# sykefi/syke-pic

Measured on AMD Instinct MI355X. Metric: IFCB images/sec, resnet50 224x224 infer step, higher is better.
Workload: dtype f16; 1 GPU; resnet50_infer_b256x1_224x224x3_50cls_head256-128; per_gpu_batch=256, global_batch=256, precision=calibrated, parallelism=dp1

## Files before the change

### include/sykepic_hip.h

```cpp
#ifndef SYKEPIC_HIP_H
#define SYKEPIC_HIP_H

#include <stdint.h>

#ifdef __cplusplus
extern "C" {
#endif

#define SPK_OK 0
#define SPK_ERR_ARG (-1)
#define SPK_ERR_HIP (-2)
#define SPK_ERR_KEY (-3)
#define SPK_ERR_UNSUPPORTED (-4)
#define SPK_ERR_STATE (-5)

#define SPK_OP_CONV 1
#define SPK_OP_MAXPOOL 2
#define SPK_OP_GAVGPOOL 3
#define SPK_OP_LINEAR 4
#define SPK_OP_DROPOUT 5
#define SPK_OP_DWCONV 6
#define SPK_OP_SE 7

#define SPK_ACT_NONE 0
// ... 135 lines not shown
int spk_op_conv_group_dgrad(const void* dy_dev, const float* w_dev, void* dx_dev, int accumulate, int n, int h, int w,
                            int c, int groups, int stride, void* hip_stream);
int spk_op_conv_group_wgrad(const void* x_dev, const void* dy_dev, float* dw_dev, int n, int h, int w, int c, int groups,
                            int stride, void* hip_stream);
int spk_op_pw_fp8(const void* x_dev, int a_fp8, const float* w_dev, void* y_dev, int out_fp8, const void* res_dev,
                  const float* bn_scale_dev, const float* bn_bias_dev, const float* gate_dev, int hw, int m_rows, int cin,
                  int cout, int act, float a_scale, float y_scale, void* hip_stream);
int spk_op_conv1x1(const void* x_dev, const float* w_dev, const float* bn_scale_dev, const float* bn_bias_dev,
                   const void* res_dev, void* y_dev, int n, int h, int w, int cin, int cout, int stride, int relu,
                   int split, int cfg, void* hip_stream);
int spk_op_conv1x1_num_configs(void);
int spk_op_conv3x3(const void* x_dev, const float* w_dev, const float* bn_scale_dev, const float* bn_bias_dev,
                   const void* res_dev, void* y_dev, int n, int h, int w, int cin, int cout, int relu, int split, int cfg,
                   void* hip_stream);
int spk_op_conv3x3_num_configs(void);
int spk_op_bottleneck(const void* x_dev, const float* w1_dev, const float* w2_dev, const float* w3_dev, const float* s1_dev,
                      const float* b1_dev, const float* s2_dev, const float* b2_dev, const float* s3_dev, const float* b3_dev,
                      void* y_dev, int n, int h, int w, int cm, int fused, int iters, float* ms_out, void* stream,
                      unsigned long long* stamps_dev ,
                      const float* wz_dev, const float* sz_dev, const float* bz_dev, void* z_dev, int coutz);
int spk_op_conv1x1_chain(const void* x, const float* w, const float* bn_scale, const float* bn_bias, const void* res,
                         void* y, const float* wz, const float* bnz_scale, const float* bnz_bias, void* z, int n, int h,
                         int wd, int cin, int cout, int coutz, int relu, int reluz, void* stream);
int spk_op_conv1x1_dual(const void* x, const float* w1, const float* s1, const float* b1, const void* x2, const float* w2,
                        const float* s2, const float* b2, void* y, int n, int ho, int wo, int cin, int h2, int w2d, int cin2,
                        int cout, int stride2, int relu, int split, int cfg, void* stream);
int spk_op_zero_sum_round(const float* w_dev, const float* mu_dev, float* out_dev, int64_t rows, int row_len,
                          int mu_period, void* stream);
int spk_op_dwconv(const void* x_dev, const float* w_dev, const float* bn_scale_dev, const float* bn_bias_dev, void* y_dev,
                  float* pool_dev, int n, int h, int w, int channels, int k, int stride, int act, int lds, void* hip_stream);
// ... 103 lines not shown
```

### syke-pic_amd/csrc/asan_driver.hip

```cpp
#include "model.h"
#include "tune_table.h"
#include <algorithm>
#include <cmath>
#include <cstdio>
#include <cstdlib>
#include <cstring>
#include <sstream>
#include <string>
#include <vector>

static int g_fail = 0;
#define EXPECT(c) do { if (!(c)) { fprintf(stderr, "asan_driver: %s:%d: %s\n", __FILE__, __LINE__, #c); ++g_fail; } } while (0)

static spk_layer_desc conv(const char* name, const char* bn, int cin, int cout, int k, int s, int p, int src, int dst,
                           int res, int relu, int child) {
  spk_layer_desc d;
  memset(&d, 0, sizeof d);
  d.kind = SPK_OP_CONV; d.cin = cin; d.cout = cout; d.k = k; d.stride = s; d.pad = p; d.relu = relu;
  d.src = src; d.dst = dst; d.res = res; d.child = child;
  snprintf(d.name, sizeof d.name, "%s", name);
  snprintf(d.bn, sizeof d.bn, "%s", bn);
  return d;
}

// ... 90 lines not shown
    spk_tune_store((TuneTag)l.tag, l.v.data(), v, true);
  }
  EXPECT(std::count(tags, tags + TUNE_NTAGS, true) == 6);
  std::vector<TuneLine> back = read_tune_lines(tmp);
  auto by_text = [](const TuneLine& x, const TuneLine& y) { return x.text < y.text; };
  std::sort(lines.begin(), lines.end(), by_text);
  std::sort(back.begin(), back.end(), by_text);
  EXPECT(back.size() == lines.size());
  for (size_t i = 0; i < lines.size() && i < back.size(); ++i) EXPECT(back[i].text == lines[i].text);

  const std::vector<std::vector<int>> fresh = {
      {2, 1, 0, 5, 9, 9, 64, 64, 3, 1, 16, 1, 0, 6, 5}, {1, 9, 9, 64, 64, 1, 0, 1, 5, -1}, {1, 9, 9, 64, 18, 18, 64, 128, 1, 2, 5, 17},
      {2, 9, 9, 64, 64, 5, 13}, {9, 9, 64, 0, 64, 5, 0}, {9, 64, 5, 2}, {81, 64, 64, 3, 1, 0, 1, 64064, 1}};
  for (int t = 0; t < (int)fresh.size(); ++t) spk_tune_store((TuneTag)t, fresh[t].data(), fresh[t].data() + kTuneSchemas[t].n_key, true);
  spk_tune_store(TUNE_DW, dk, &one, true);
  EXPECT(read_tune_lines(tmp).size() == lines.size() + fresh.size());
  use_cache(tmp.c_str());
  for (int t = 0; t < (int)fresh.size(); ++t) {
    int v[2] = {-1000, -1000};
    EXPECT(spk_tune_find((TuneTag)t, fresh[t].data(), v));
    for (int i = 0; i < kTuneSchemas[t].n_val; ++i) EXPECT(v[i] == fresh[t][kTuneSchemas[t].n_key + i]);
  }
  EXPECT(look(TUNE_DW, {0, 64, 28, 28, 240, 5, 1}) == -1000);
  EXPECT(spk_tune_detail::table().map.size() == lines.size() + fresh.size());
  remove(tmp.c_str());
}

int main(int argc, char** argv) {
  int ndev = 0;
  const bool gpu = hipGetDeviceCount(&ndev) == hipSuccess && ndev > 0;
  printf("asan_driver: %d GPU(s)\n", gpu ? ndev : 0);

  spk_model* m = nullptr;
  EXPECT(spk_model_create(nullptr, 0, 3, 10, 0, &m) != SPK_OK);
  EXPECT(strlen(spk_last_error()) > 0);
  EXPECT(spk_model_num_params(nullptr) == 0);
  spk_model_destroy(nullptr);
  {
    float f[4] = {0};
// ... 69 lines not shown
  }

  const std::string path = std::string(getenv("TMPDIR") ? getenv("TMPDIR") : "/tmp") + "/spk_asan_tune_cache.txt";
  std::string seed = argc > 1 ? argv[1] : std::string(argv[0]);
  if (argc <= 1) seed = seed.substr(0, seed.find_last_of('/') + 1) + "../../../sykepic_hip/tune_seed_gfx950.txt";
  tuner_table_checks(path + ".rt", seed);
  std::string fixture;
  if (FILE* f = fopen(path.c_str(), "w")) {
    fprintf(f, "conv 0 1 1 256 14 14 256 256 3 1 16 0 0 4 3\n");
    fprintf(f, "pw1x1 2 14 14 256 1024 1 1 1 256 7\n");
    fprintf(f, "pw2 1 14 14 256 28 28 512 1024 1 2 256 5\n");
    fprintf(f, "c3 1 14 14 256 256 256 2\n");
    fprintf(f, "chain 14 14 256 0 256 64 0\n");
    fprintf(f, "bneck 14 256 8 1\n");
    fprintf(f, "wgrad 6272 256 256 3 1 0 13 128128 1\n");
    fprintf(f, "pw1x1 2 14 14 256 2048 1 1 1 256 99999\n");
    fprintf(f, "pw1x1 2 14 14 256 2048 1 1 1 256 -2\n");
    fprintf(f, "pw2 1 14 14 256 28 28 512 2048 1 2 256 %d\n", kPwNumCfgs);
    fprintf(f, "pw2 1 14 14 256 28 28 512 2048 1 2 256 -1\n");
    fprintf(f, "c3 1 14 14 256 512 256 %d\n", kC3NumCfgs);
    fprintf(f, "chain 14 14 256 0 512 64 2\n");
    fprintf(f, "bneck 28 128 8 3\n");
    fprintf(f, "c3 1 14 14\n");
    fprintf(f, "bneck 28 128 8\n");
    fprintf(f, "bneck 28 128 8 1 1\n");
    fprintf(f, "chain 14 14 256 0 512 64 1x\n");
    fprintf(f, "wgrad 6272 256 512 3 1 0 13 128128 99999999999\n");
    fprintf(f, "# bneck 28 128 8 2\n#bneck 28 128 8 2\n");
    fprintf(f, "conv x y z\n\n,,,,\nbneck\nbneckx 28 128 8 2\n");
    for (int i = 0; i < 3000; ++i) fputc('9', f);
// ... 3 lines not shown
    fprintf(f, "wgrad 1 2 3\n");
    fprintf(f, "c3 2 7 7 512 512 128 13");
    fclose(f);
    for (const TuneLine& l : read_tune_lines(path)) fixture += l.text;
  }
  use_cache(path.c_str());
  int dma = -1;
  EXPECT(look(TUNE_CONV, {0, 1, 1, 256, 14, 14, 256, 256, 3, 1, 16, 0, 0}, &dma) == 4 && dma == 3);
  EXPECT(look(TUNE_PW1, {2, 14, 14, 256, 1024, 1, 1, 1, 256}) == 7);
  EXPECT(look(TUNE_PW2, {1, 14, 14, 256, 28, 28, 512, 1024, 1, 2, 256}) == 5);
  EXPECT(look(TUNE_C3, {1, 14, 14, 256, 256, 256}) == 2);
  EXPECT(look(TUNE_CHAIN, {14, 14, 256, 0, 256, 64}) == 0);
  EXPECT(look(TUNE_BNECK, {14, 256, 8}) == 1);
  EXPECT(look(TUNE_WGRAD, {6272, 256, 256, 3, 1, 0, 13, 128128}) == 1);
  EXPECT(look(TUNE_C3, {2, 7, 7, 512, 512, 128}) == 13);
  EXPECT(look(TUNE_PW1, {2, 14, 14, 256, 2048, 1, 1, 1, 256}) == -1000);
  EXPECT(look(TUNE_PW2, {1, 14, 14, 256, 28, 28, 512, 2048, 1, 2, 256}) == -1000);
  EXPECT(look(TUNE_C3, {1, 14, 14, 256, 512, 256}) == -1000);
  EXPECT(look(TUNE_CHAIN, {14, 14, 256, 0, 512, 64}) == -1000);
  EXPECT(look(TUNE_BNECK, {28, 128, 8}) == -1000);
  EXPECT(look(TUNE_WGRAD, {6272, 256, 512, 3, 1, 0, 13, 128128}) == -1000);
  EXPECT(spk_tune_detail::table().map.size() == 8);
  setenv("SPK_AUTOTUNE", "0", 1);
  const int n = 1, h = 8, wd = 8, cin = 128, cout = 128, M = n * h * wd;
  bf16_t *x = nullptr, *y = nullptr, *wp = nullptr;
  float* sb = nullptr;
  if (gpu) {
    EXPECT(hipMalloc(&x, (size_t)M * cin * 2) == hipSuccess && hipMalloc(&y, (size_t)M * 256 * 2) == hipSuccess);
    EXPECT(hipMalloc(&wp, (size_t)256 * 9 * cin * 4) == hipSuccess && hipMalloc(&sb, (size_t)2 * 256 * 4) == hipSuccess);
    (void)hipMemset(x, 0, (size_t)M * cin * 2);
    (void)hipMemset(wp, 0, (size_t)256 * 9 * cin * 4);
    (void)hipMemset(sb, 0, (size_t)2 * 256 * 4);
  }
  ConvArgs a;
  memset(&a, 0, sizeof a);
  a.cfg = a.dma = -1; a.cls_ph = a.cls_pw = -1;
  a.x = x; a.w = wp; a.y = y; a.scale = sb; a.bias = sb ? sb + cout : nullptr;
// ... 29 lines not shown
```

### syke-pic_amd/csrc/model.h

```cpp
#pragma once
#include "../../include/sykepic_hip.h"
#include "spk_common.h"

#include <string>
#include <unordered_map>
#include <vector>

enum ParamKind { PK_CONV_W = 1, PK_BN_W, PK_BN_B, PK_BN_MEAN, PK_BN_VAR, PK_BN_NBT, PK_FC_W, PK_FC_B,
                 PK_SE_W, PK_SE_B };

struct Param {
  std::string key;
  int kind = 0, layer = -1, dtype = 0, ndim = 0;
  int64_t shape[4] = {1, 1, 1, 1};
  int64_t numel = 0;
  bool trainable = false;
  int requires_grad = 0;
  int group = -1;
  size_t off = 0;
  long step = 0;
  double mu_product = 1.0;
};

struct TDim {
// ... 2 lines not shown
  int c_log = 0;
};

struct Layer {
  spk_layer_desc d;
  int mode = 0;
  int groups = 1;
  int kpad = 0;
  int p_w = -1, p_g = -1, p_b = -1, p_mean = -1, p_var = -1, p_nbt = -1;
  int p_w2 = -1, p_b2 = -1;
  int cin_p = 0, cout_p = 0;
  size_t wpack_off = 0, sb_off = 0;
  size_t wpw_off = 0;
  bool pw_ok = false;
  bool c3_ok = false;
  int dual_src = -1;
  int fused_into = -1;
  bool dual_ok = false;
  size_t wdual_off = 0;
  size_t sdual_off = 0;
  int chain_next = -1;
  int chained_by = -1;
  bool chained_now_h[2] = {false, false};
  int bn_c2 = -1, bn_c3 = -1;
  int bn_head = -1;
  bool bneck_now_h[2] = {false, false};
  bool btail_now_h[2] = {false, false};
  size_t mu_off = 0;
  int gate_conv = -1;
  int gate_from = -1;
// ... 154 lines not shown
```

### syke-pic_amd/csrc/model.hip

```cpp
#include "../../include/sykepic_hip.h"
#include "spk_common.h"
#include "model.h"
#include "tune_table.h"

#include <algorithm>
#include <cmath>
#include <cstdio>
#include <cstdlib>
#include <cstring>

static thread_local std::string g_err;

void spk_set_error(const std::string& s) { g_err = s; }

#define HIP_TRY(expr)                                                                   \
  do {                                                                                  \
    hipError_t e_ = (expr);                                                             \
    if (e_ != hipSuccess) {                                                             \
      spk_set_error(std::string(#expr) + ": " + hipGetErrorString(e_));                 \
      return SPK_ERR_HIP;                                                               \
    }                                                                                   \
  } while (0)

#define SPK_TRY(expr)              \
// ... 258 lines not shown
      L.wpack_off = wpack;
      wpack += (size_t)2 * L.cout_p * L.kpad;
      L.pw_ok = L.mode == CONV_MODE_GENERIC && L.d.k == 1 && L.d.pad == 0 && L.cin_p == L.d.cin && L.cout_p == L.d.cout &&
                L.d.cin % 64 == 0 && L.d.cout % 64 == 0 && L.kpad == L.d.cin && L.d.relu != SPK_ACT_HSWISH;
      if (L.pw_ok) {
        L.wpw_off = wpack;
        wpack += (size_t)2 * L.d.cout * L.d.cin;
      }
      L.c3_ok = L.mode == CONV_MODE_GENERIC && L.d.k == 3 && L.d.stride == 1 && L.d.pad == 1 && L.cin_p == L.d.cin &&
                L.cout_p == L.d.cout && L.d.cin % 64 == 0 &&
                (L.d.cout % 256 == 0 || (L.bn_head >= 0 && L.d.cout % 128 == 0)) && L.d.relu != SPK_ACT_HSWISH;
      if (L.c3_ok || (L.bn_head >= 0 && L.d.k == 3)) {
        L.wpw_off = wpack;
        wpack += (size_t)2 * L.d.cout * 9 * L.d.cin;
      }
    } else {
      continue;
    }
    L.sb_off = sb;
    sb += (size_t)2 * L.cout_p;
  }
  size_t wdual = 0, sdual = 0;
  for (size_t i = 0; i < m->layers.size(); ++i) {
    Layer& L = m->layers[i];
    if (L.d.kind != SPK_OP_CONV || !L.pw_ok || L.d.res < 0 || L.d.stride != 1) continue;
    for (size_t j = 0; j < m->layers.size(); ++j) {
      Layer& D = m->layers[j];
      if (D.d.kind != SPK_OP_CONV || D.d.dst != L.d.res || !D.pw_ok || !D.side_branch || D.d.relu != 0 || D.d.res >= 0 ||
          D.d.cout != L.d.cout || D.fused_into >= 0)
        continue;
// ... 297 lines not shown
      r = pack_stem3(m, L);
    else if (L.mode == CONV_MODE_GENERIC && (L.cin_p != L.d.cin || L.cout_p != L.d.cout))
      r = spk_launch_pack_padded(wsrc, m->wpack + L.wpack_off, L.d.cout, L.d.k * L.d.k, L.d.cin, L.cout_p,
                                 L.cin_p, m->infer_dt, layer_split(m, L), m->stream);
    else
      r = spk_launch_pack_weights(wsrc, m->wpack + L.wpack_off, L.d.cout, L.d.k, L.d.k, L.d.cin,
                                  L.mode, m->infer_dt, layer_split(m, L), m->stream);
    if (r) return fail(SPK_ERR_HIP, "pack_weights launch failed");
    if (L.pw_ok && m->infer_dt == DT_F16 &&
        spk_launch_pack_pw(wsrc, nullptr, m->wpack + L.wpw_off, L.d.cout, L.d.cin, DT_F16, layer_split(m, L) ? 2 : 1,
                           m->stream))
      return fail(SPK_ERR_HIP, "pack_pw launch failed");
    if ((L.c3_ok || (L.bn_head >= 0 && L.d.k == 3)) && m->infer_dt == DT_F16 &&
        spk_launch_pack_c3(wsrc, m->wpack + L.wpw_off, L.d.cout, L.d.cin, layer_split(m, L) ? 2 : 1, m->stream))
      return fail(SPK_ERR_HIP, "pack_c3 launch failed");
  }
  {
    size_t tmp_floats = 0;
    for (Layer& L : m->layers) {
      L.dual_ok = false;
      if (L.dual_src < 0 || m->infer_dt != DT_F16) continue;
      const Layer& D = m->layers[L.dual_src];
      if ((layer_split(m, L) != 0) != (layer_split(m, D) != 0)) continue;
      tmp_floats = std::max(tmp_floats, (size_t)L.d.cout * (L.d.cin + D.d.cin));
    }
    float* wcat = nullptr;
    float* mucat = nullptr;
    bool dual_zs = false;
    for (const Layer& L : m->layers) dual_zs |= L.dual_src >= 0 && layer_zero_sum(m, L) && layer_zero_sum(m, m->layers[L.dual_src]);
    if (tmp_floats) HIP_TRY(hipMalloc((void**)&wcat, tmp_floats * 4 * (dual_zs ? 2 : 1) + (dual_zs ? 16384 * 4 : 0)));
// ... 568 lines not shown
    return SPK_OK;
  }
  static const bool use_c3 = !getenv("SPK_C3") || atoi(getenv("SPK_C3")) != 0;
  if (use_c3 && L.c3_ok && a.dt == DT_F16 && !a.res_lo && !a.y_lo && !a.cin_s && !a.cout_s) {
    C3Args q;
    memset(&q, 0, sizeof q);
    q.x = a.x; q.wp = m->wpack + L.wpw_off; q.y = a.y; q.scale = a.scale; q.shift = a.bias;
    q.N = nb; q.H = in.h; q.W = in.w; q.Cin = a.Cin; q.Cout = a.Cout; q.M = a.M; q.relu = a.relu; q.dt = DT_F16;
    q.nb = a.splitw ? 2 : 1;
    q.x_bytes = a.x_bytes; q.y_bytes = (unsigned)((size_t)a.M * a.Cout * 2);
    q.wp_bytes = (unsigned)((size_t)a.Cout * 9 * a.Cin * 2 * q.nb);
    q.res = a.res;
    const int r = spk_conv3x3_launch(q, m->stream);
    if (r == 0) return SPK_OK;
    if (r != -3) return fail(SPK_ERR_HIP, std::string("3x3 conv launch failed for ") + L.d.name);
  }
  if (spk_conv_launch(a, L.mode, m->stream, nullptr))
    return fail(SPK_ERR_HIP, std::string("conv launch failed for ") + L.d.name);
  return SPK_OK;
}

static int dw_forced() {
  static const int v = getenv("SPK_DW_LDS") ? atoi(getenv("SPK_DW_LDS")) : -1;
  return v;
}

template <class F>
static int dw_choose(int et, int nb, int h, int w, int c, int k, int s, hipStream_t st, F run, const int* chunks) {
  if (dw_forced() >= 0) {
    const int v = dw_forced();
// ... 648 lines not shown
```

### syke-pic_amd/csrc/ops_abi.hip

```cpp
#include "model.h"
#include "train_effnet.h"

#include <algorithm>
#include <cstring>
#include <vector>

static int ofail(int code, const std::string& msg) {
  spk_set_error(msg);
  return code;
}

namespace {
struct Scratch {
  std::vector<void*> p;
  ~Scratch() { for (void* q : p) (void)hipFree(q); }
  template <typename T> T* get(size_t count) {
    void* q = nullptr;
    if (hipMalloc(&q, (count ? count : 1) * sizeof(T)) != hipSuccess) return nullptr;
    p.push_back(q);
    return (T*)q;
  }
};
bool stem_shape(int cin, int cout, int k, int stride, int pad) {
  return cin <= 4 && k == 7 && stride == 2 && pad == 3 && cout == 64;
// ... 353 lines not shown
    memset(&q, 0, sizeof q);
    q.x = (const bf16_t*)x; q.wp = wp; q.y = (bf16_t*)y; q.scale = bn_scale; q.shift = bn_bias;
    q.N = n; q.H = h; q.W = wd; q.Cin = cin; q.Cout = cout; q.M = M; q.relu = relu; q.dt = DT_F16; q.nb = split ? 2 : 1;
    q.x_bytes = (unsigned)((size_t)M * cin * 2);
    q.y_bytes = (unsigned)((size_t)M * cout * 2);
    q.wp_bytes = (unsigned)((size_t)cout * 9 * cin * 2 * q.nb);
    q.res = (const bf16_t*)res;
    r = spk_c3_launch(q, cfg, s);
    if (r == -3) return ofail(SPK_ERR_UNSUPPORTED, "this configuration does not fit the problem");
  }
  if (r) return ofail(SPK_ERR_HIP, "conv3x3 launch failed");
  if (hipStreamSynchronize(s) != hipSuccess) return ofail(SPK_ERR_HIP, "conv3x3 kernel failed");
  return SPK_OK;
}
extern "C" int spk_op_conv3x3_num_configs(void) { return spk_c3_num_configs(); }

extern "C" int spk_op_bottleneck(const void* x, const float* w1, const float* w2, const float* w3, const float* s1,
                                 const float* b1, const float* s2, const float* b2, const float* s3, const float* b3, void* y,
                                 int n, int h, int wd, int cm, int fused, int iters, float* ms_out, void* stream,
                                 unsigned long long* stamps_dev, const float* wz, const float* sz, const float* bz, void* z,
                                 int coutz) {
  if (!x || !w1 || !w2 || !w3 || !s1 || !b1 || !s2 || !b2 || !s3 || !b3 || !y || n < 1 || h < 1 || wd < 1 || x == y)
    return ofail(SPK_ERR_ARG, "op_bottleneck: bad arguments");
  if (cm % 64) return ofail(SPK_ERR_UNSUPPORTED, "mid channels must be a multiple of 64");
  hipStream_t s = (hipStream_t)stream;
  const int c4 = 4 * cm, M = n * h * wd;
  if ((size_t)M * c4 * 2 >= 0x80000000ull) return ofail(SPK_ERR_UNSUPPORTED, "op_bottleneck: an operand of 2 GiB or more");
  Scratch sc;
  bf16_t* p1 = sc.get<bf16_t>((size_t)cm * c4);
  bf16_t* p2 = sc.get<bf16_t>((size_t)9 * cm * cm);
// ... 643 lines not shown
```

### syke-pic_amd/csrc/spk_common.h

```cpp
#pragma once
#include <hip/hip_runtime.h>
#include <stdint.h>
#include <stddef.h>
#include <atomic>

static inline bool spk_lds_limit_once(std::atomic<unsigned long long>& mask, const void* kernel, int bytes) {
  int dev = 0;
  if (hipGetDevice(&dev) != hipSuccess) return false;
  const unsigned long long bit = dev >= 0 && dev < 64 ? 1ull << dev : 0ull;
  if (mask.load(std::memory_order_acquire) & bit) return true;
  if (hipFuncSetAttribute(kernel, hipFuncAttributeMaxDynamicSharedMemorySize, bytes) != hipSuccess) return false;
  mask.fetch_or(bit, std::memory_order_release);
  return true;
}

typedef unsigned short bf16_t;

typedef __attribute__((ext_vector_type(8))) __bf16 bf16x8_t;
typedef __attribute__((ext_vector_type(4))) float f32x4_t;
typedef __attribute__((ext_vector_type(4))) unsigned int u32x4_t;
typedef __attribute__((ext_vector_type(2))) unsigned int u32x2_t;

__device__ __forceinline__ float bf16_to_f32(bf16_t v) {
  return __builtin_bit_cast(float, ((unsigned int)v) << 16);
// ... 143 lines not shown
struct C3Args {
  const bf16_t* x;
  const bf16_t* wp;
  bf16_t* y;
  const float* scale;
  const float* shift;
  int N, H, W, Cin, Cout, M;
  int relu, dt, nb;
  unsigned int x_bytes, y_bytes, wp_bytes;
  const bf16_t* res;
};
int spk_c3_num_configs();
int spk_c3_launch(const C3Args& a, int cfg, hipStream_t s);
int spk_launch_pack_c3(const float* w_ohwi, bf16_t* out, int cout, int cin, int nb, hipStream_t s);
int spk_conv3x3_launch(const C3Args& a, hipStream_t s);

struct BneckArgs {
  const bf16_t* x;
  bf16_t* y;
  const bf16_t* w1;
  const bf16_t* w2;
  const bf16_t* w3;
  const float *s1, *b1, *s2, *b2, *s3, *b3;
  int N, H, W, C4, CM;
  unsigned int x_bytes;
  const bf16_t* y1;
  const bf16_t* wz;
  bf16_t* z;
  const float *sz, *bz;
  int Coutz;
// ... 140 lines not shown
```

### syke-pic_amd/csrc/tune_table.h

```cpp
#pragma once
#include <hip/hip_runtime.h>
#include <algorithm>
#include <array>
#include <climits>
#include <cstdio>
#include <cstdlib>
#include <cstring>
#include <map>
#include <mutex>

constexpr int kPwNumCfgs = 18;
constexpr int kC3NumCfgs = 14;

struct TuneSchema { const char* tag; int n_key, n_pos, n_val, val_min, val_max; };
enum TuneTag { TUNE_CONV, TUNE_PW1, TUNE_PW2, TUNE_C3, TUNE_CHAIN, TUNE_BNECK, TUNE_WGRAD, TUNE_DW, TUNE_NTAGS };
constexpr TuneSchema kTuneSchemas[TUNE_NTAGS] = {
    {"conv", 13, 3, 2, INT_MIN, INT_MAX},
    {"pw1x1", 9, 8, 1, -1, kPwNumCfgs - 1},
    {"pw2", 11, 10, 1, 0, kPwNumCfgs - 1},
    {"c3", 6, 5, 1, -1, kC3NumCfgs - 1},
    {"chain", 6, 5, 1, 0, 1},
    {"bneck", 3, 2, 1, 0, 2},
    {"wgrad", 8, -1, 1, INT_MIN, INT_MAX},
    {nullptr, 7, -1, 1, 0, 1},
};

inline const char* spk_tune_cache_path() {
  const char* e = getenv("SPK_TUNE_CACHE");
  return e && *e && strcmp(e, "off") ? e : nullptr;
}
inline bool spk_autotune_on() {
  static const bool v = !getenv("SPK_AUTOTUNE") || atoi(getenv("SPK_AUTOTUNE")) != 0;
  return v;
}
inline int spk_tune_log() {
  static const int v = getenv("SPK_TUNE_LOG") ? (atoi(getenv("SPK_TUNE_LOG")) > 1 ? atoi(getenv("SPK_TUNE_LOG")) : 1) : 0;
  return v;
}

// ... 136 lines not shown
```

### syke-pic_amd/sykepic_hip/lib.py

```python

import ctypes as C
import os
from pathlib import Path

_HERE = Path(__file__).resolve().parent
LIB_PATH = Path(os.environ.get("SYKEPIC_HIP_LIB", _HERE / "libsykepic_hip.so"))


class LayerDesc(C.Structure):
    _fields_ = [
        ("kind", C.c_int32), ("cin", C.c_int32), ("cout", C.c_int32), ("k", C.c_int32),
        ("stride", C.c_int32), ("pad", C.c_int32), ("relu", C.c_int32), ("src", C.c_int32),
        ("dst", C.c_int32), ("res", C.c_int32), ("child", C.c_int32), ("p", C.c_float),
        ("name", C.c_char * 96), ("bn", C.c_char * 96),
    ]


class OptimDesc(C.Structure):
    _fields_ = [
        ("kind", C.c_int32), ("lr", C.c_float * 3), ("beta1", C.c_float), ("beta2", C.c_float),
        ("eps", C.c_float), ("weight_decay", C.c_float), ("momentum", C.c_float),
        ("grad_scale", C.c_float), ("alpha", C.c_float), ("momentum_decay", C.c_float),
        ("lr_decay", C.c_float), ("initial_accumulator_value", C.c_float),
    ]
# ... 101 lines not shown
    "spk_op_mbconv_eval_geometry": (C.c_int, [C.c_int] * 5 + [C.POINTER(C.c_int)]),
    "spk_op_linear": (C.c_int, [_P] * 4 + [C.c_int] * 3 + [_P]),
    "spk_op_linear_backward": (C.c_int, [_P] * 6 + [C.c_int] * 4 + [_P]),
    "spk_op_softmax": (C.c_int, [_P, _P, C.c_int, C.c_int, C.c_float, _P]),
    "spk_op_cross_entropy": (C.c_int, [_P, _P, C.c_int, C.c_int, _P, _P, _P]),
    "spk_op_cross_entropy_ex": (C.c_int, [_P, _P, C.c_int, C.c_int, _P, C.c_float, _P, _P, _P, _P]),
    "spk_op_cross_entropy_pair": (C.c_int, [_P, _P, _P, C.c_float, C.c_int, C.c_int, _P, C.c_float, _P, _P, _P, _P]),
    "spk_op_maxpool": (C.c_int, [_P] * 3 + [C.c_int] * 8 + [_P]),
    "spk_op_maxpool_backward": (C.c_int, [_P] * 3 + [C.c_int] * 8 + [_P]),
    "spk_op_gavgpool": (C.c_int, [_P, _P] + [C.c_int] * 4 + [_P]),
    "spk_op_gavgpool_backward": (C.c_int, [_P, _P] + [C.c_int] * 3 + [_P]),
    "spk_op_conv1x1": (C.c_int, [_P, _P, _P, _P, _P, _P] + [C.c_int] * 9 + [_P]),
    "spk_op_conv1x1_num_configs": (C.c_int, []),
    "spk_op_conv3x3": (C.c_int, [_P, _P, _P, _P, _P, _P] + [C.c_int] * 8 + [_P]),
    "spk_op_conv3x3_num_configs": (C.c_int, []),
    "spk_op_bottleneck": (C.c_int, [_P] * 11 + [C.c_int] * 6 + [_P, _P, _P] + [_P] * 4 + [C.c_int]),
    "spk_preprocess_rois": (C.c_int, [_P, C.c_int64, _P, C.c_int, C.c_int, C.c_int, C.c_int, _P, _P]),
    "spk_predict_rows": (C.c_int, [_P, C.c_int, C.c_int, _P, C.c_float, _P, _P, _P]),
    "spk_augment_batch": (C.c_int, [_P, _P, _P, C.c_int, C.c_int, C.c_int, C.c_int, _P, C.c_int, _P, _P]),
    "spk_mix_batch": (C.c_int, [_P, _P] + [C.c_int] * 7 + [C.c_float, C.c_float] + [C.c_int] * 4 + [_P]),
    "spk_model_profile_infer": (C.c_int, [_P, _P, C.c_int, C.c_int, C.c_int, C.c_int, C.c_int,
                                          C.c_int, C.POINTER(LayerTime), C.c_int]),
    "spk_model_profile_train": (C.c_int, [_P, _P, C.c_int, C.c_int, C.c_int, C.c_int, C.c_int, _P, _P,
                                          C.c_int, C.POINTER(LayerTime), C.c_int]),
}

GRAD_READY_FN = C.CFUNCTYPE(None, C.c_void_p, C.c_int, C.c_int64, C.c_int64)

_lib = None

# ... 69 lines not shown
```

### syke-pic_amd/sykepic_hip/ops.py

```python

import contextlib
import ctypes as C

import torch

from . import lib


def _nhwc(t):
    return t.permute(0, 2, 3, 1).contiguous()


def _nchw(t_nhwc):
    return t_nhwc.permute(0, 3, 1, 2)


def _p(t):
    return C.c_void_p(t.data_ptr()) if t is not None else None


def _stream(dev):
    return C.c_void_p(torch.cuda.current_stream(dev).cuda_stream)


# ... 213 lines not shown

def conv3x3(x, weight, bn_scale, bn_bias, relu=True, split=False, cfg=0, res=None):
    so = lib.load()
    dev = x.device
    n, cin, h, w = x.shape
    cout = weight.shape[0]
    xh = x.half().permute(0, 2, 3, 1).contiguous()
    y = torch.full((n, h, w, cout), float("nan"), dtype=torch.float16, device=dev)
    wk = weight.float().permute(0, 2, 3, 1).contiguous()
    rh = res.half().permute(0, 2, 3, 1).contiguous() if res is not None else None
    with torch.cuda.device(dev):
        lib.check(so.spk_op_conv3x3(_p(xh), _p(wk), _p(bn_scale.float().contiguous()), _p(bn_bias.float().contiguous()),
                                    _p(rh) if rh is not None else None, _p(y), n, h, w, cin, cout, int(bool(relu)), int(bool(split)), int(cfg),
                                    _stream(dev)))
    return y.permute(0, 3, 1, 2)


def bottleneck(x, w1, w2, w3, bn1, bn2, bn3, fused=True, iters=0, stamps=None, wz=None, bnz=None):
    import ctypes as C
    so = lib.load()
    dev = x.device
    n, c4, h, w = x.shape
    cm = w1.shape[0]
    xh = x.half().permute(0, 2, 3, 1).contiguous()
    y = torch.full((n, h, w, c4), float("nan"), dtype=torch.float16, device=dev)
    k1 = w1.float().reshape(cm, c4).contiguous()
    k2 = w2.float().permute(0, 2, 3, 1).contiguous()
    k3 = w3.float().reshape(c4, cm).contiguous()
    vecs = [t.float().contiguous() for pair in (bn1, bn2, bn3) for t in pair]
    ms = C.c_float(0.0)
# ... 430 lines not shown
```

Measured before the change: 79410 images/s.

## Add direct 3x3 conv kernel for 64-channel layers with autotuned selection

Adds a specialized direct 3x3 convolution kernel for 64-in/64-out stride-1 f16 layers. It keeps the whole packed weight panel in LDS, works through pixel tiles persistently, and reuses row loads across horizontal taps with DPP lane shifts. The model dispatch autotunes this kernel against the existing implicit-GEMM path per shape and picks it only when it is clearly faster, caching the choice in the tune table. The aim is to cut the redundant input loads and weight traffic of the generic path on ResNet50's first-stage 3x3 convs, at the cost of added code complexity and autotune time.

```diff
diff --git a/include/sykepic_hip.h b/include/sykepic_hip.h
--- a/include/sykepic_hip.h
+++ b/include/sykepic_hip.h
@@ -173,6 +173,10 @@
                    const void* res_dev, void* y_dev, int n, int h, int w, int cin, int cout, int relu, int split, int cfg,
                    void* hip_stream);
 int spk_op_conv3x3_num_configs(void);
+int spk_op_conv3x3_direct(const void* x_dev, const float* w_dev, const float* bn_scale_dev, const float* bn_bias_dev,
+                          const void* res_dev, void* y_dev, int n, int h, int w, int cin, int cout, int stride, int relu,
+                          int split, int cfg, int iters, float* ms_out, void* stream);
+int spk_op_conv3x3_direct_num_configs(void);
 int spk_op_bottleneck(const void* x_dev, const float* w1_dev, const float* w2_dev, const float* w3_dev, const float* s1_dev,
                       const float* b1_dev, const float* s2_dev, const float* b2_dev, const float* s3_dev, const float* b3_dev,
                       void* y_dev, int n, int h, int w, int cm, int fused, int iters, float* ms_out, void* stream,
diff --git a/syke-pic_amd/csrc/asan_driver.hip b/syke-pic_amd/csrc/asan_driver.hip
--- a/syke-pic_amd/csrc/asan_driver.hip
+++ b/syke-pic_amd/csrc/asan_driver.hip
@@ -128,15 +128,20 @@
       {2, 9, 9, 64, 64, 5, 13}, {9, 9, 64, 0, 64, 5, 0}, {9, 64, 5, 2}, {81, 64, 64, 3, 1, 0, 1, 64064, 1}};
   for (int t = 0; t < (int)fresh.size(); ++t) spk_tune_store((TuneTag)t, fresh[t].data(), fresh[t].data() + kTuneSchemas[t].n_key, true);
   spk_tune_store(TUNE_DW, dk, &one, true);
-  EXPECT(read_tune_lines(tmp).size() == lines.size() + fresh.size());
+  const int d3_fresh[] = {9, 9, 1, 5, kD3NumCfgs - 1};
+  spk_tune_store(TUNE_D3, d3_fresh, d3_fresh + kTuneSchemas[TUNE_D3].n_key, true);
+  EXPECT(read_tune_lines(tmp).size() == lines.size() + fresh.size() + 1);
   use_cache(tmp.c_str());
+  EXPECT(look(TUNE_D3, {9, 9, 1, 5}) == kD3NumCfgs - 1);
+  EXPECT(look(TUNE_D3, {9, 9, 1, 8}) == kD3NumCfgs - 1);
+  EXPECT(look(TUNE_D3, {9, 9, 0, 5}) == -1000);
   for (int t = 0; t < (int)fresh.size(); ++t) {
     int v[2] = {-1000, -1000};
     EXPECT(spk_tune_find((TuneTag)t, fresh[t].data(), v));
     for (int i = 0; i < kTuneSchemas[t].n_val; ++i) EXPECT(v[i] == fresh[t][kTuneSchemas[t].n_key + i]);
   }
   EXPECT(look(TUNE_DW, {0, 64, 28, 28, 240, 5, 1}) == -1000);
-  EXPECT(spk_tune_detail::table().map.size() == lines.size() + fresh.size());
+  EXPECT(spk_tune_detail::table().map.size() == lines.size() + fresh.size() + 1);
   remove(tmp.c_str());
 }
 
@@ -236,6 +241,8 @@
     fprintf(f, "chain 14 14 256 0 256 64 0\n");
     fprintf(f, "bneck 14 256 8 1\n");
     fprintf(f, "wgrad 6272 256 256 3 1 0 13 128128 1\n");
+    fprintf(f, "d3 56 56 0 128 -1\n");
+    fprintf(f, "d3 56 56 1 128 %d\n", kD3NumCfgs);
     fprintf(f, "pw1x1 2 14 14 256 2048 1 1 1 256 99999\n");
     fprintf(f, "pw1x1 2 14 14 256 2048 1 1 1 256 -2\n");
     fprintf(f, "pw2 1 14 14 256 28 28 512 2048 1 2 256 %d\n", kPwNumCfgs);
@@ -269,13 +276,15 @@
   EXPECT(look(TUNE_BNECK, {14, 256, 8}) == 1);
   EXPECT(look(TUNE_WGRAD, {6272, 256, 256, 3, 1, 0, 13, 128128}) == 1);
   EXPECT(look(TUNE_C3, {2, 7, 7, 512, 512, 128}) == 13);
+  EXPECT(look(TUNE_D3, {56, 56, 0, 128}) == -1);
+  EXPECT(look(TUNE_D3, {56, 56, 1, 128}) == -1000);
   EXPECT(look(TUNE_PW1, {2, 14, 14, 256, 2048, 1, 1, 1, 256}) == -1000);
   EXPECT(look(TUNE_PW2, {1, 14, 14, 256, 28, 28, 512, 2048, 1, 2, 256}) == -1000);
   EXPECT(look(TUNE_C3, {1, 14, 14, 256, 512, 256}) == -1000);
   EXPECT(look(TUNE_CHAIN, {14, 14, 256, 0, 512, 64}) == -1000);
   EXPECT(look(TUNE_BNECK, {28, 128, 8}) == -1000);
   EXPECT(look(TUNE_WGRAD, {6272, 256, 512, 3, 1, 0, 13, 128128}) == -1000);
-  EXPECT(spk_tune_detail::table().map.size() == 8);
+  EXPECT(spk_tune_detail::table().map.size() == 9);
   setenv("SPK_AUTOTUNE", "0", 1);
   const int n = 1, h = 8, wd = 8, cin = 128, cout = 128, M = n * h * wd;
   bf16_t *x = nullptr, *y = nullptr, *wp = nullptr;
diff --git a/syke-pic_amd/csrc/conv_d3.hip b/syke-pic_amd/csrc/conv_d3.hip
--- /dev/null
+++ b/syke-pic_amd/csrc/conv_d3.hip
@@ -0,0 +1,336 @@
+#include "spk_common.h"
+#include "tune_table.h"
+#include <cstdio>
+#include <cstdlib>
+#include <cstring>
+
+namespace {
+
+typedef __attribute__((address_space(3))) const unsigned char* lds_u8_t;
+typedef __attribute__((address_space(3))) const u32x4_t* lds_u32x4_t;
+typedef __attribute__((address_space(3))) const f32x4_t* lds_f32x4_t;
+
+typedef __attribute__((ext_vector_type(2))) float f32x2_t;
+typedef __attribute__((ext_vector_type(2))) _Float16 f16x2_t;
+__device__ __forceinline__ unsigned int pack2_f16(float lo, float hi) {
+  const f32x2_t v = {lo, hi};
+  return __builtin_bit_cast(unsigned int, __builtin_convertvector(v, f16x2_t));
+}
+
+struct D3Geom {
+  int H, W, HW, M;
+  float rcp_hw, rcp_w;
+};
+
+constexpr int kC = 64;
+constexpr int kKS = 18;
+constexpr int kCH = 2 * 2048;
+constexpr int kPanel = kKS * kCH;
+constexpr int kLds = kPanel + 2 * kC * 4;
+
+template <int MT, int WAVES, int PA, int WPE, bool HAS_RES>
+__global__ __launch_bounds__(WAVES * 64, WPE) void conv_d3_kernel(C3Args a, D3Geom gm, int m_tiles) {
+  constexpr bool REUSE = PA == 0;
+  static_assert(REUSE || kKS % PA == 0, "the register sets rotate with the K steps of a tile");
+  constexpr int DT = DT_F16;
+  constexpr int NPAIR = 2, NT = 4, BN = kC;
+  constexpr int WPX = MT * 16, BM = WAVES * WPX, T = WAVES * 64;
+
+  extern __shared__ __attribute__((aligned(16))) unsigned char smem[];
+  const int tid = threadIdx.x;
+  const int lane = tid & 63;
+  const int wave = __builtin_amdgcn_readfirstlane(tid >> 6);
+  const int g = lane >> 4, p = lane & 15;
+
+  const __amdgpu_buffer_rsrc_t rx = __builtin_amdgcn_make_buffer_rsrc((void*)a.x, 0, a.x_bytes, 0x00020000);
+  const __amdgpu_buffer_rsrc_t ry = __builtin_amdgcn_make_buffer_rsrc((void*)a.y, 0, a.y_bytes, 0x00020000);
+  const __amdgpu_buffer_rsrc_t rr = __builtin_amdgcn_make_buffer_rsrc((void*)a.res, 0, HAS_RES ? a.y_bytes : 0, 0x00020000);
+
+  int mt = (int)((long)blockIdx.x * m_tiles / (int)gridDim.x);
+  const int mt_end = (int)((long)(blockIdx.x + 1) * m_tiles / (int)gridDim.x);
+
+  unsigned char* const sW = smem;
+  float* const sScale = (float*)(smem + kPanel);
+
+  struct TileState { unsigned off[MT]; unsigned msk[MT]; unsigned ml[MT]; unsigned mr[MT]; };
+  auto tile_state = [&](int tile, TileState& st) {
+#pragma unroll
+    for (int m = 0; m < MT; ++m) {
+      const int px = tile * BM + wave * WPX + m * 16 + p;
+      const bool ok = tile < mt_end && px < gm.M;
+      int img = (int)((float)px * gm.rcp_hw);
+      int rem = px - img * gm.HW;
+      if (rem < 0) rem += gm.HW;
+      else if (rem >= gm.HW) rem -= gm.HW;
+      int row = (int)((float)rem * gm.rcp_w);
+      int col = rem - row * gm.W;
+      if (col < 0) { col += gm.W; --row; }
+      else if (col >= gm.W) { col -= gm.W; ++row; }
+      const unsigned cm = (col > 0 ? 1u : 0u) | 2u | (col < gm.W - 1 ? 4u : 0u);
+      unsigned mk = (row > 0 ? cm : 0u) | (cm << 3) | (row < gm.H - 1 ? cm << 6 : 0u);
+      st.msk[m] = ok ? mk : 0u;
+      st.ml[m] = ok && col > 0 ? ~0u : 0u;
+      st.mr[m] = ok && col < gm.W - 1 ? ~0u : 0u;
+      st.off[m] = ok ? (unsigned)px * (unsigned)(kC * 2) + (unsigned)g * 16u : 0x80000000u;
+    }
+  };
+
+  f32x4_t acc[MT][NT];
+  u32x4_t xa[REUSE ? 1 : PA][MT];
+  struct RowFrag { u32x4_t c[2], e[2]; };
+  RowFrag rows[REUSE ? 3 : 1][MT];
+
+  const int row_bytes = gm.W * (kC * 2);
+  auto load_a = [&](u32x4_t (&dst)[MT], const TileState& st, int u) {
+    const int t = u >> 1;
+    const int tap_off = (t / 3 - 1) * row_bytes + (t % 3 - 1) * (kC * 2);
+#pragma unroll
+    for (int m = 0; m < MT; ++m) {
+      const unsigned vo = (st.msk[m] >> t) & 1u ? st.off[m] + (unsigned)tap_off : 0x80000000u;
+      dst[m] = __builtin_amdgcn_raw_buffer_load_b128(rx, vo, (u & 1) * 64, 0);
+    }
+  };
+  auto load_row = [&](RowFrag (&dst)[MT], const TileState& st, int dy) {
+#pragma unroll
+    for (int m = 0; m < MT; ++m) {
+      const bool rok = (st.msk[m] >> (3 * dy + 1)) & 1u;
+      const unsigned vo = rok ? st.off[m] + (unsigned)((dy - 1) * row_bytes) : 0x80000000u;
+      const unsigned eo = p == 0 ? (rok && st.ml[m] ? vo - (unsigned)(kC * 2) : 0x80000000u)
+                                 : (p == 15 && rok && st.mr[m] ? vo + (unsigned)(kC * 2) : 0x80000000u);
+#pragma unroll
+      for (int h = 0; h < 2; ++h) {
+        dst[m].c[h] = __builtin_amdgcn_raw_buffer_load_b128(rx, vo, h * 64, 0);
+        dst[m].e[h] = __builtin_amdgcn_raw_buffer_load_b128(rx, eo, h * 64, 0);
+      }
+    }
+  };
+  auto tap_frag = [&](u32x4_t (&f)[MT], const RowFrag (&r)[MT], const TileState& st, int dxi, int h) {
+#pragma unroll
+    for (int m = 0; m < MT; ++m) {
+      if (dxi == 1) { f[m] = r[m].c[h]; continue; }
+#pragma unroll
+      for (int k = 0; k < 4; ++k) {
+        const unsigned s = dxi == 0 ? __builtin_amdgcn_update_dpp(r[m].e[h][k], r[m].c[h][k], 0x111, 0xf, 0xf, false)
+                                    : __builtin_amdgcn_update_dpp(r[m].e[h][k], r[m].c[h][k], 0x101, 0xf, 0xf, false);
+        f[m][k] = s & (dxi == 0 ? st.ml[m] : st.mr[m]);
+      }
+    }
+  };
+  auto init_acc = [&]() {
+#pragma unroll
+    for (int m = 0; m < MT; ++m)
+#pragma unroll
+      for (int t = 0; t < NT; ++t) acc[m][t] = f32x4_t{0.f, 0.f, 0.f, 0.f};
+  };
+  struct Frag { u32x4_t w[2]; };
+  Frag fr[2];
+  auto load_frag = [&](Frag& f, lds_u8_t q) {
+    f.w[0] = *(lds_u32x4_t)(q);
+    f.w[1] = *(lds_u32x4_t)(q + 1024);
+  };
+  auto compute = [&](lds_u8_t base, lds_u8_t next, const u32x4_t (&x)[MT]) {
+#pragma unroll
+    for (int P = 0; P < NPAIR; ++P) {
+      if (P + 1 < NPAIR) load_frag(fr[(P + 1) & 1], base + (P + 1) * 2048 + lane * 16);
+      else load_frag(fr[0], next + lane * 16);
+#pragma unroll
+      for (int m = 0; m < MT; ++m) {
+        acc[m][2 * P] = mfma16<DT>(fr[P & 1].w[0], x[m], acc[m][2 * P]);
+        acc[m][2 * P + 1] = mfma16<DT>(fr[P & 1].w[1], x[m], acc[m][2 * P + 1]);
+      }
+      __builtin_amdgcn_sched_group_barrier(0x100, 2, 0);
+      __builtin_amdgcn_sched_group_barrier(0x008, 2 * MT, 0);
+    }
+  };
+
+  u32x4_t rv[HAS_RES ? MT : 1][NPAIR];
+  const float out_max = 65504.f;
+  const float relu_floor = a.relu == 1 ? 0.f : -out_max;
+  auto epilogue = [&](const unsigned (&yoff)[MT], const unsigned (&yoff_next)[MT]) {
+#pragma unroll
+    for (int m = 0; m < MT; ++m) {
+#pragma unroll
+      for (int P = 0; P < NPAIR; ++P) {
+        lds_f32x4_t sp = (lds_f32x4_t)(sScale + P * 32 + 8 * g);
+        asm volatile("" : "+v"(sp));
+        const f32x4_t sc0 = sp[0], sc1 = sp[1], sh0 = sp[BN / 4], sh1 = sp[BN / 4 + 1];
+        float v[8];
+#pragma unroll
+        for (int r = 0; r < 4; ++r) {
+          v[r] = __builtin_fmaf(acc[m][2 * P][r], sc0[r], sh0[r]);
+          v[4 + r] = __builtin_fmaf(acc[m][2 * P + 1][r], sc1[r], sh1[r]);
+        }
+        if (HAS_RES) {
+          const u32x4_t q = rv[HAS_RES ? m : 0][P];
+#pragma unroll
+          for (int j = 0; j < 4; ++j) {
+            v[2 * j] += lo_f32<DT>(q[j]);
+            v[2 * j + 1] += hi_f32<DT>(q[j]);
+          }
+          rv[HAS_RES ? m : 0][P] = __builtin_amdgcn_raw_buffer_load_b128(rr, yoff_next[m] + P * 64, 0, 0);
+        }
+#pragma unroll
+        for (int j = 0; j < 8; ++j) v[j] = __builtin_amdgcn_fmed3f(v[j], relu_floor, out_max);
+        u32x4_t ov;
+#pragma unroll
+        for (int j = 0; j < 4; ++j) ov[j] = pack2_f16(v[2 * j], v[2 * j + 1]);
+        __builtin_amdgcn_raw_buffer_store_b128(ov, ry, yoff[m] + P * 64, 0, 0);
+      }
+    }
+  };
+  auto prologue_like_an_epilogue = [&](const unsigned (&yoff)[MT]) {
+    const __amdgpu_buffer_rsrc_t rnull = __builtin_amdgcn_make_buffer_rsrc((void*)a.y, 0, 0, 0x00020000);
+#pragma unroll
+    for (int m = 0; m < MT; ++m)
+#pragma unroll
+      for (int P = 0; P < NPAIR; ++P) {
+        if (HAS_RES) rv[HAS_RES ? m : 0][P] = __builtin_amdgcn_raw_buffer_load_b128(rr, yoff[m] + P * 64, 0, 0);
+        __builtin_amdgcn_raw_buffer_store_b128(u32x4_t{0, 0, 0, 0}, rnull, yoff[m] + P * 64, 0, 0);
+      }
+  };
+
+  for (int c = tid; c < BN; c += T) {
+    sScale[c] = a.scale ? a.scale[c] : 1.f;
+    sScale[BN + c] = a.shift ? a.shift[c] : 0.f;
+  }
+  {
+    constexpr int RD = kPanel / (T * 16);
+    static_assert(kPanel % (T * 16) == 0, "whole copy rounds");
+    u32x4_t wv[RD];
+#pragma unroll
+    for (int r = 0; r < RD; ++r) wv[r] = *(const u32x4_t*)((const unsigned char*)a.wp + r * (T * 16) + tid * 16);
+#pragma unroll
+    for (int r = 0; r < RD; ++r) *(u32x4_t*)(sW + r * (T * 16) + tid * 16) = wv[r];
+  }
+
+  TileState cur, nxt;
+  tile_state(mt, cur);
+  tile_state(mt + 1, nxt);
+  if constexpr (REUSE) {
+#pragma unroll
+    for (int dy = 0; dy < 3; ++dy) load_row(rows[dy], cur, dy);
+  } else {
+#pragma unroll
+    for (int u = 0; u < PA; ++u) load_a(xa[u], cur, u);
+  }
+  prologue_like_an_epilogue(cur.off);
+  __syncthreads();
+  const lds_u8_t sWl = (lds_u8_t)sW;
+  load_frag(fr[0], sWl + lane * 16);
+  while (mt < mt_end) {
+    init_acc();
+    lds_u8_t sbase = sWl;
+#pragma unroll
+    for (int u = 0; u < kKS; ++u) {
+      lds_u8_t snext = u + 1 < kKS ? sbase + kCH : sWl;
+      asm volatile("" : "+v"(snext));
+      if constexpr (REUSE) {
+        const int dy = u / 6, dxi = (u % 6) / 2;
+        u32x4_t f[MT];
+        tap_frag(f, rows[dy], cur, dxi, u & 1);
+        compute(sbase, snext, f);
+        if (u % 6 == 5) load_row(rows[dy], nxt, dy);
+      } else {
+        compute(sbase, snext, xa[u % PA]);
+        if (u + PA < kKS) load_a(xa[u % PA], cur, u + PA);
+        else load_a(xa[u % PA], nxt, u + PA - kKS);
+      }
+      sbase = snext;
+    }
+    epilogue(cur.off, nxt.off);
+    ++mt;
+    cur = nxt;
+    tile_state(mt + 1, nxt);
+  }
+}
+
+int d3_cu_count() {
+  static std::atomic<int> cus[64];
+  int dev = 0;
+  if (hipGetDevice(&dev) != hipSuccess || dev < 0 || dev >= 64) return 256;
+  int n = cus[dev].load(std::memory_order_relaxed);
+  if (n > 0) return n;
+  if (hipDeviceGetAttribute(&n, hipDeviceAttributeMultiprocessorCount, dev) != hipSuccess || n <= 0) {
+    (void)hipGetLastError();
+    n = 256;
+  }
+  cus[dev].store(n, std::memory_order_relaxed);
+  return n;
+}
+
+template <int MT, int WAVES, int PA, int WPE>
+int launch_k(const C3Args& a, int bpc, hipStream_t s) {
+  constexpr int BM = WAVES * MT * 16;
+  const int m_tiles = (a.M + BM - 1) / BM;
+  void (*k)(C3Args, D3Geom, int) = a.res ? conv_d3_kernel<MT, WAVES, PA, WPE, true> : conv_d3_kernel<MT, WAVES, PA, WPE, false>;
+  static std::atomic<unsigned long long> attr[2];
+  if (!spk_lds_limit_once(attr[a.res != nullptr], (const void*)k, kLds)) return -1;
+  D3Geom gm;
+  gm.H = a.H; gm.W = a.W; gm.HW = a.H * a.W; gm.M = a.M;
+  gm.rcp_hw = 1.0f / (float)gm.HW;
+  gm.rcp_w = 1.0f / (float)a.W;
+  int grid = d3_cu_count() * bpc;
+  if (grid > m_tiles) grid = m_tiles;
+  hipLaunchKernelGGL(k, dim3(grid), dim3(WAVES * 64), kLds, s, a, gm, m_tiles);
+  return hipGetLastError() == hipSuccess ? 0 : -1;
+}
+
+}
+
+int spk_d3_num_configs() { return kD3NumCfgs; }
+
+int spk_d3_launch(const C3Args& a, int cfg, hipStream_t s) {
+  if (a.dt != DT_F16 || a.nb != 1 || (a.relu != 0 && a.relu != 1) || a.Cin != kC || a.Cout != kC || a.M <= 0 || a.M != a.N * a.H * a.W) return -3;
+  if ((size_t)a.x_bytes >= 0x80000000ull || (size_t)a.y_bytes >= 0x80000000ull) return -3;
+  switch (cfg) {
+    case 0: return launch_k<2, 4, 0, 2>(a, 2, s);
+    case 1: return launch_k<1, 4, 0, 2>(a, 2, s);
+    case 2: return launch_k<1, 8, 0, 4>(a, 2, s);
+    case 3: return launch_k<2, 8, 0, 2>(a, 1, s);
+    case 4: return launch_k<2, 4, 6, 2>(a, 2, s);
+    case 5: return launch_k<2, 4, 18, 2>(a, 2, s);
+    default: return -3;
+  }
+}
+
+namespace {
+int d3_mode() {
+  static const int v = getenv("SPK_D3") ? atoi(getenv("SPK_D3")) : 1;
+  return v;
+}
+}
+
+int spk_conv3x3_d3_launch(const ConvArgs& a, const C3Args& q, hipStream_t s) {
+  if (d3_mode() == 0) return spk_conv_launch(a, CONV_MODE_GENERIC, s, nullptr);
+  const int key[] = {q.H, q.W, q.res != nullptr, q.N};
+  int choice = -1;
+  const bool found = spk_tune_find(TUNE_D3, key, &choice);
+  if (d3_mode() == 2 && (!found || choice < 0)) choice = 0;
+  if (!found && spk_autotune_on()) {
+    SpkLaunchTimer timer;
+    if (!timer.ok) return -1;
+    float t_igemm = 1e30f, t_d3 = 1e30f;
+    int best_d3 = -1;
+    for (int cfg = (d3_mode() == 2 ? 0 : -1); cfg < kD3NumCfgs; ++cfg) {
+      auto run = [&]() { return cfg < 0 ? spk_conv_launch(a, CONV_MODE_GENERIC, s, nullptr) : spk_d3_launch(q, cfg, s); };
+      if (run()) continue;
+      float ms = 0.f;
+      if (!timer.time(s, 3, run, &ms)) continue;
+      if (spk_tune_log() > 1)
+        fprintf(stderr, "[spk d3 cand] N%d %dx%d res%d: %s %d %.1f us\n", q.N, q.H, q.W, q.res != nullptr,
+                cfg < 0 ? "igemm" : "d3", cfg, ms * 1000.f / 3.f);
+      if (cfg < 0) t_igemm = ms;
+      else if (ms < t_d3) { t_d3 = ms; best_d3 = cfg; }
+    }
+    choice = best_d3 >= 0 && t_d3 < 0.92f * t_igemm ? best_d3 : -1;
+    spk_tune_store(TUNE_D3, key, &choice, d3_mode() != 2);
+    if (spk_tune_log())
+      fprintf(stderr, "[spk tune d3] N%d %dx%d res%d: %s %d (%.1f us)\n", q.N, q.H, q.W, q.res != nullptr,
+              choice < 0 ? "igemm" : "d3", choice, (choice < 0 ? t_igemm : t_d3) * 1000.f / 3.f);
+  }
+  if (choice >= 0) {
+    if (spk_d3_launch(q, choice, s) == 0) return 0;
+    (void)hipGetLastError();
+  }
+  return spk_conv_launch(a, CONV_MODE_GENERIC, s, nullptr);
+}
diff --git a/syke-pic_amd/csrc/model.h b/syke-pic_amd/csrc/model.h
--- a/syke-pic_amd/csrc/model.h
+++ b/syke-pic_amd/csrc/model.h
@@ -40,6 +40,8 @@
   size_t wpw_off = 0;
   bool pw_ok = false;
   bool c3_ok = false;
+  bool d3_ok = false;
+  size_t wd3_off = 0;
   int dual_src = -1;
   int fused_into = -1;
   bool dual_ok = false;
diff --git a/syke-pic_amd/csrc/model.hip b/syke-pic_amd/csrc/model.hip
--- a/syke-pic_amd/csrc/model.hip
+++ b/syke-pic_amd/csrc/model.hip
@@ -296,6 +296,12 @@
         L.wpw_off = wpack;
         wpack += (size_t)2 * L.d.cout * 9 * L.d.cin;
       }
+      L.d3_ok = L.mode == CONV_MODE_GENERIC && L.d.k == 3 && L.d.stride == 1 && L.d.pad == 1 && L.cin_p == L.d.cin &&
+                L.cout_p == L.d.cout && L.d.cin == 64 && L.d.cout == 64 && L.kpad == 9 * L.d.cin && L.d.relu != SPK_ACT_HSWISH;
+      if (L.d3_ok) {
+        L.wd3_off = wpack;
+        wpack += (size_t)L.d.cout * 9 * L.d.cin;
+      }
     } else {
       continue;
     }
@@ -623,6 +629,9 @@
     if ((L.c3_ok || (L.bn_head >= 0 && L.d.k == 3)) && m->infer_dt == DT_F16 &&
         spk_launch_pack_c3(wsrc, m->wpack + L.wpw_off, L.d.cout, L.d.cin, layer_split(m, L) ? 2 : 1, m->stream))
       return fail(SPK_ERR_HIP, "pack_c3 launch failed");
+    if (L.d3_ok && m->infer_dt == DT_F16 && !layer_split(m, L) &&
+        spk_launch_pack_pw(wsrc, nullptr, m->wpack + L.wd3_off, L.d.cout, 9 * L.d.cin, DT_F16, 1, m->stream))
+      return fail(SPK_ERR_HIP, "pack_pw (3x3 panel) launch failed");
   }
   {
     size_t tmp_floats = 0;
@@ -1221,6 +1230,16 @@
     const int r = spk_conv3x3_launch(q, m->stream);
     if (r == 0) return SPK_OK;
     if (r != -3) return fail(SPK_ERR_HIP, std::string("3x3 conv launch failed for ") + L.d.name);
+  }
+  if (L.d3_ok && a.dt == DT_F16 && !a.splitw && !a.res_lo && !a.y_lo && !a.cin_s && !a.cout_s && !a.pool_y) {
+    C3Args q;
+    memset(&q, 0, sizeof q);
+    q.x = a.x; q.wp = m->wpack + L.wd3_off; q.y = a.y; q.scale = a.scale; q.shift = a.bias; q.res = a.res;
+    q.N = nb; q.H = in.h; q.W = in.w; q.Cin = a.Cin; q.Cout = a.Cout; q.M = a.M; q.relu = a.relu; q.dt = DT_F16; q.nb = 1;
+    q.x_bytes = a.x_bytes; q.y_bytes = (unsigned)((size_t)a.M * a.Cout * 2);
+    if (spk_conv3x3_d3_launch(a, q, m->stream))
+      return fail(SPK_ERR_HIP, std::string("3x3 conv launch failed for ") + L.d.name);
+    return SPK_OK;
   }
   if (spk_conv_launch(a, L.mode, m->stream, nullptr))
     return fail(SPK_ERR_HIP, std::string("conv launch failed for ") + L.d.name);
diff --git a/syke-pic_amd/csrc/ops_abi.hip b/syke-pic_amd/csrc/ops_abi.hip
--- a/syke-pic_amd/csrc/ops_abi.hip
+++ b/syke-pic_amd/csrc/ops_abi.hip
@@ -1,5 +1,6 @@
 #include "model.h"
 #include "train_effnet.h"
+#include "tune_table.h"
 
 #include <algorithm>
 #include <cstring>
@@ -391,6 +392,52 @@
   return SPK_OK;
 }
 extern "C" int spk_op_conv3x3_num_configs(void) { return spk_c3_num_configs(); }
+
+extern "C" int spk_op_conv3x3_direct(const void* x, const float* w_ohwi, const float* bn_scale, const float* bn_bias,
+                                     const void* res, void* y, int n, int h, int wd, int cin, int cout, int stride, int relu,
+                                     int split, int cfg, int iters, float* ms_out, void* stream) {
+  if (!x || !w_ohwi || !bn_scale || !bn_bias || !y || n < 1 || h < 1 || wd < 1 || (stride != 1 && stride != 2) || iters < 0)
+    return ofail(SPK_ERR_ARG, "op_conv3x3_direct: bad arguments");
+  if (cin % 64 || cout % 64) return ofail(SPK_ERR_UNSUPPORTED, "channels must be multiples of 64");
+  if (cfg >= 0 && (cin != 64 || cout != 64 || stride != 1 || split))
+    return ofail(SPK_ERR_UNSUPPORTED, "this configuration does not fit the problem");
+  hipStream_t s = (hipStream_t)stream;
+  const int ho = (h - 1) / stride + 1, wo = (wd - 1) / stride + 1, M = n * ho * wo;
+  if ((size_t)n * h * wd * cin * 2 >= 0x80000000ull || (size_t)M * cout * 2 >= 0x80000000ull)
+    return ofail(SPK_ERR_UNSUPPORTED, "op_conv3x3_direct: an operand of 2 GiB or more (split the batch)");
+  Scratch sc;
+  bf16_t* wp = sc.get<bf16_t>((size_t)2 * cout * 9 * cin);
+  if (!wp) return ofail(SPK_ERR_HIP, "hipMalloc failed");
+  ConvArgs a;
+  memset(&a, 0, sizeof a);
+  a.cfg = a.dma = -1;
+  a.cls_ph = a.cls_pw = -1;
+  a.x = (const bf16_t*)x; a.w = wp; a.y = (bf16_t*)y; a.scale = bn_scale; a.bias = bn_bias; a.res = (const bf16_t*)res;
+  a.N = n; a.H = h; a.W = wd; a.Cin = cin; a.Ho = ho; a.Wo = wo; a.Cout = cout;
+  a.kh = a.kw = 3; a.stride = stride; a.pad = 1; a.M = M; a.K = 9 * cin; a.relu = relu; a.dt = DT_F16; a.splitw = split != 0;
+  a.x_bytes = (unsigned)((size_t)n * h * wd * cin * 2);
+  a.w_bytes = (unsigned)((size_t)cout * 9 * cin * 2 * (split ? 2 : 1));
+  C3Args q;
+  memset(&q, 0, sizeof q);
+  q.x = a.x; q.wp = wp; q.y = a.y; q.scale = bn_scale; q.shift = bn_bias; q.res = a.res;
+  q.N = n; q.H = h; q.W = wd; q.Cin = cin; q.Cout = cout; q.M = M; q.relu = relu; q.dt = DT_F16; q.nb = 1;
+  q.x_bytes = a.x_bytes; q.y_bytes = (unsigned)((size_t)M * cout * 2);
+  if (cfg < 0) O_TRY(spk_launch_pack_weights(w_ohwi, wp, cout, 3, 3, cin, CONV_MODE_GENERIC, DT_F16, split != 0, s), "pack_weights");
+  else O_TRY(spk_launch_pack_pw(w_ohwi, nullptr, wp, cout, 9 * cin, DT_F16, 1, s), "pack_pw");
+  auto run = [&]() { return cfg < 0 ? spk_conv_launch(a, CONV_MODE_GENERIC, s, nullptr) : spk_d3_launch(q, cfg, s); };
+  const int r = run();
+  if (r == -3) return ofail(SPK_ERR_UNSUPPORTED, "this configuration does not fit the problem");
+  if (r) return ofail(SPK_ERR_HIP, "conv3x3_direct launch failed");
+  if (hipStreamSynchronize(s) != hipSuccess) return ofail(SPK_ERR_HIP, "conv3x3_direct kernel failed");
+  if (iters > 0 && ms_out) {
+    SpkLaunchTimer timer;
+    float ms = 0.f;
+    if (!timer.ok || !timer.time(s, iters, run, &ms)) return ofail(SPK_ERR_HIP, "conv3x3_direct timing failed");
+    *ms_out = ms / (float)iters;
+  }
+  return SPK_OK;
+}
+extern "C" int spk_op_conv3x3_direct_num_configs(void) { return spk_d3_num_configs(); }
 
 extern "C" int spk_op_bottleneck(const void* x, const float* w1, const float* w2, const float* w3, const float* s1,
                                  const float* b1, const float* s2, const float* b2, const float* s3, const float* b3, void* y,
diff --git a/syke-pic_amd/csrc/spk_common.h b/syke-pic_amd/csrc/spk_common.h
--- a/syke-pic_amd/csrc/spk_common.h
+++ b/syke-pic_amd/csrc/spk_common.h
@@ -181,6 +181,10 @@
 int spk_c3_launch(const C3Args& a, int cfg, hipStream_t s);
 int spk_launch_pack_c3(const float* w_ohwi, bf16_t* out, int cout, int cin, int nb, hipStream_t s);
 int spk_conv3x3_launch(const C3Args& a, hipStream_t s);
+
+int spk_d3_num_configs();
+int spk_d3_launch(const C3Args& a, int cfg, hipStream_t s);
+int spk_conv3x3_d3_launch(const ConvArgs& a, const C3Args& q, hipStream_t s);
 
 struct BneckArgs {
   const bf16_t* x;
diff --git a/syke-pic_amd/csrc/tune_table.h b/syke-pic_amd/csrc/tune_table.h
--- a/syke-pic_amd/csrc/tune_table.h
+++ b/syke-pic_amd/csrc/tune_table.h
@@ -11,9 +11,10 @@
 
 constexpr int kPwNumCfgs = 18;
 constexpr int kC3NumCfgs = 14;
+constexpr int kD3NumCfgs = 6;
 
 struct TuneSchema { const char* tag; int n_key, n_pos, n_val, val_min, val_max; };
-enum TuneTag { TUNE_CONV, TUNE_PW1, TUNE_PW2, TUNE_C3, TUNE_CHAIN, TUNE_BNECK, TUNE_WGRAD, TUNE_DW, TUNE_NTAGS };
+enum TuneTag { TUNE_CONV, TUNE_PW1, TUNE_PW2, TUNE_C3, TUNE_CHAIN, TUNE_BNECK, TUNE_WGRAD, TUNE_DW, TUNE_D3, TUNE_NTAGS };
 constexpr TuneSchema kTuneSchemas[TUNE_NTAGS] = {
     {"conv", 13, 3, 2, INT_MIN, INT_MAX},
     {"pw1x1", 9, 8, 1, -1, kPwNumCfgs - 1},
@@ -23,6 +24,7 @@
     {"bneck", 3, 2, 1, 0, 2},
     {"wgrad", 8, -1, 1, INT_MIN, INT_MAX},
     {nullptr, 7, -1, 1, 0, 1},
+    {"d3", 4, 3, 1, -1, kD3NumCfgs - 1},
 };
 
 inline const char* spk_tune_cache_path() {
diff --git a/syke-pic_amd/sykepic_hip/lib.py b/syke-pic_amd/sykepic_hip/lib.py
--- a/syke-pic_amd/sykepic_hip/lib.py
+++ b/syke-pic_amd/sykepic_hip/lib.py
@@ -139,6 +139,8 @@
     "spk_op_conv1x1_num_configs": (C.c_int, []),
     "spk_op_conv3x3": (C.c_int, [_P, _P, _P, _P, _P, _P] + [C.c_int] * 8 + [_P]),
     "spk_op_conv3x3_num_configs": (C.c_int, []),
+    "spk_op_conv3x3_direct": (C.c_int, [_P, _P, _P, _P, _P, _P] + [C.c_int] * 10 + [_P, _P]),
+    "spk_op_conv3x3_direct_num_configs": (C.c_int, []),
     "spk_op_bottleneck": (C.c_int, [_P] * 11 + [C.c_int] * 6 + [_P, _P, _P] + [_P] * 4 + [C.c_int]),
     "spk_preprocess_rois": (C.c_int, [_P, C.c_int64, _P, C.c_int, C.c_int, C.c_int, C.c_int, _P, _P]),
     "spk_predict_rows": (C.c_int, [_P, C.c_int, C.c_int, _P, C.c_float, _P, _P, _P]),
diff --git a/syke-pic_amd/sykepic_hip/ops.py b/syke-pic_amd/sykepic_hip/ops.py
--- a/syke-pic_amd/sykepic_hip/ops.py
+++ b/syke-pic_amd/sykepic_hip/ops.py
@@ -251,6 +251,30 @@
                                     _p(rh) if rh is not None else None, _p(y), n, h, w, cin, cout, int(bool(relu)), int(bool(split)), int(cfg),
                                     _stream(dev)))
     return y.permute(0, 3, 1, 2)
+
+
+def conv3x3_direct_num_configs():
+    return int(lib.load().spk_op_conv3x3_direct_num_configs())
+
+
+def conv3x3_direct(x, weight, bn_scale, bn_bias, relu=True, split=False, cfg=0, res=None, stride=1, iters=0):
+    import ctypes as C
+    so = lib.load()
+    dev = x.device
+    n, cin, h, w = x.shape
+    cout = weight.shape[0]
+    ho, wo = (h - 1) // stride + 1, (w - 1) // stride + 1
+    xh = x.half().permute(0, 2, 3, 1).contiguous()
+    y = torch.full((n, ho, wo, cout), float("nan"), dtype=torch.float16, device=dev)
+    wk = weight.float().permute(0, 2, 3, 1).contiguous()
+    rh = res.half().permute(0, 2, 3, 1).contiguous() if res is not None else None
+    ms = C.c_float(0.0)
+    with torch.cuda.device(dev):
+        lib.check(so.spk_op_conv3x3_direct(_p(xh), _p(wk), _p(bn_scale.float().contiguous()), _p(bn_bias.float().contiguous()),
+                                           _p(rh) if rh is not None else None, _p(y), n, h, w, cin, cout, int(stride),
+                                           int(bool(relu)), int(bool(split)), int(cfg), int(iters), C.byref(ms), _stream(dev)))
+    y = y.permute(0, 3, 1, 2)
+    return (y, float(ms.value)) if iters > 0 else y
 
 
 def bottleneck(x, w1, w2, w3, bn1, bn2, bn3, fused=True, iters=0, stamps=None, wz=None, bnz=None):
```

New measurement: 81310 images/s, median of 6. +2.4%, better.
